# MirceaKitsune/python_raytracer

Measured on AMD Instinct MI355X. Metric: Mrays/s (primary+bounce), higher is better.
Workload: dtype f64; 1 GPU; mods/default 3840x2160 spp8 max_bounces8 (BASELINE config 3/4); width=3840, height=2160, samples=8, primary_rays=62725130, bounce_rays=75192856, partition=(x ^ y) % 1, traversed=True, fast_draws=32, frames_in_flight=1, scene_flow=pre-selected camera chunks (fixture), rng_retraced_rays=0, rng_table=static seeds: draw table + ray table built once before the timed region, reused

## Files before the change

### python_raytracer_amd/_native.py

```python
import ctypes as C
import os
import subprocess

HERE = os.path.dirname(os.path.abspath(__file__))
ROOT = os.path.dirname(HERE)
DIAG = os.environ.get("VRT_DIAG", "0") not in ("", "0")
DIAG_HIST = os.environ.get("VRT_DIAG", "0") == "2"
SO_OVERRIDE = os.environ.get("VRT_SO", "")
SO_PATH = SO_OVERRIDE or os.path.join(HERE, ("_vrt_diaghist.so" if DIAG_HIST else "_vrt_diag.so") if DIAG else "_vrt.so")
UNITS = [os.path.join(HERE, "csrc", f) for f in ("vrt_kernels.hip", "vrt_surface.hip")]
PHYSICS_UNITS = [os.path.join(HERE, "csrc", "vrt_physics.hip")]
PHYSICS_DRAWS_UNITS = [os.path.join(HERE, "csrc", "vrt_physics_draws.hip")]
PHYSICS_RUN_UNITS = [os.path.join(HERE, "csrc", "vrt_physics_run.hip")]
SOURCES = UNITS + PHYSICS_UNITS + PHYSICS_DRAWS_UNITS + PHYSICS_RUN_UNITS + \
    [os.path.join(HERE, "csrc", f) for f in ("vrt_math.h", "vrt_math_consts.h", "vrt_physics_common.h")]
SOURCES.append(os.path.join(ROOT, "include", "vrt.h"))
HIPCC = os.environ.get("HIPCC", "/opt/rocm/bin/hipcc")
HIPCC_FLAGS = ["-O3", "--offload-arch=gfx950", "-ffp-contract=off", "-std=c++17", "-fPIC", "-shared"] + \
    (["-DVRT_DIAG"] if DIAG else []) + (["-DVRT_DIAG_HIST"] if DIAG_HIST else [])

ABI_VERSION = 9
SCENE_TABLE_IS_IDENTITY = 1
SCENE_LAYOUT_DENSE = 2
ERR_WORKSPACE = -3
# ... 291 lines not shown
    L.vrt_diag_launch_census.argtypes = [C.c_int, C.c_char_p, C.c_int, C.POINTER(i64)]
    if L.vrt_abi_version() != ABI_VERSION:
        raise ImportError("python_raytracer_amd/_vrt.so has ABI version %d, expected %d"
                          % (L.vrt_abi_version(), ABI_VERSION))
    _lib = L
    return L


EXPORTS = ["vrt_abi_version", "vrt_status_string", "vrt_last_hip_error", "vrt_device_count", "vrt_release_caches", "vrt_voxel_offset",
           "vrt_max_samples", "vrt_plan_bytes", "vrt_plan_build", "vrt_workspace_bytes", "vrt_render_tile",
           "vrt_views_workspace_bytes", "vrt_render_views",
           "vrt_first_hit", "vrt_first_hit_views_workspace_bytes", "vrt_first_hit_views", "vrt_cast_rays",
           "vrt_shade_workspace_bytes", "vrt_shade_rays", "vrt_path_workspace_bytes", "vrt_path_rays", "vrt_pixel_rays",
           "vrt_draw_table_bytes", "vrt_draw_table_build", "vrt_ray_table_bytes", "vrt_ray_table_build",
           "vrt_pow_memo_create", "vrt_occupancy_build", "vrt_canvas_blit", "vrt_world_tables_bytes", "vrt_world_tables_build",
           "vrt_trace_workspace_bytes", "vrt_trace_rays", "vrt_rng_draws",
           "vrt_synth_volume", "vrt_profile_begin", "vrt_profile_begin_kinds", "vrt_profile_end", "vrt_select_chunks", "vrt_voxelize",
           "vrt_hit_owners", "vrt_hit_surfaces", "vrt_edit_models", "vrt_stamp_model", "vrt_physics_tick",
           "vrt_physics_tick_draws", "vrt_physics_run"]


PLAN_FIELDS = ("launches", "pool", "wt_on", "trav_words", "bm_window", "ct_cells", "n_materials", "dyn_bytes", "static_bytes")
PLAN_PROBE_FIELDS = ("wt_on", "trav_words", "dyn_bytes", "static_bytes", "groups_per_cu")


def last_plan():
    L = lib()
    n = L.vrt_diag_last_plan((C.c_int64 * 1)(), 0)
    if n < 0:
        check(n, "vrt_diag_last_plan")
    buf = (C.c_int64 * n)()
    L.vrt_diag_last_plan(buf, n)
    w = [int(v) for v in buf]
    plan = dict(zip(PLAN_FIELDS, w))
    k = len(PLAN_FIELDS) + 1
    plan["probes"] = [dict(zip(PLAN_PROBE_FIELDS, w[k + 5 * i:k + 5 * i + 5])) for i in range(w[len(PLAN_FIELDS)])]
    return plan


VARIANT_INPUTS = ("record", "list", "list_seed", "pool", "resmode", "deep", "per_pixel", "wt_on", "keys", "trav_words", "bm_window",
                  "big_scene", "tile_heads", "occ", "lookup", "defer_visit")
VARIANT_DEFAULTS = {**dict.fromkeys(VARIANT_INPUTS, 0), "bm_window": -1, "defer_visit": 1}


def march_variant(**inputs):
    unknown = set(inputs) - set(VARIANT_INPUTS)
    if unknown:
        raise TypeError("unknown inputs: %s" % sorted(unknown))
    words = (C.c_int32 * len(VARIANT_INPUTS))(*[int({**VARIANT_DEFAULTS, **inputs}[k]) for k in VARIANT_INPUTS])
    name, effects = C.create_string_buffer(128), (C.c_int32 * 3)()
    status = lib().vrt_diag_march_variant(words, len(VARIANT_INPUTS), name, len(name), effects)
    return (status, name.value.decode(), tuple(effects)) if status == 0 else (status, None, None)


def launch_census():
    L = lib()
    name, count = C.create_string_buffer(128), C.c_int64(0)
    census, row, n = {}, 0, 1
    while row < n:
# ... 16 lines not shown
```

### python_raytracer_amd/csrc/vrt_kernels.hip

```cpp
#include <hip/hip_runtime.h>
#include <stdint.h>
#include <stdio.h>
#include <stdlib.h>
#include <string.h>

#include <atomic>
#include <mutex>
#include <vector>

#include "../../include/vrt.h"
#include "vrt_math.h"

#pragma clang fp contract(off)

#define VRT_WAVE 64
#define VRT_BLOCK 256

static thread_local int g_last_hip_error = 0;
#define HIP_TRY(expr)                                   \
    do {                                                \
        hipError_t e__ = (expr);                        \
        if (e__ != hipSuccess) {                        \
            g_last_hip_error = (int)e__;                \
            return VRT_ERR_HIP;                         \
// ... 832 lines not shown
    double step, life, bounces, energy;
    int nm4x, nm4y, nm4z;
    uint32_t entry;
    uint32_t boff;
    uint32_t color;
    int ndraw, resnaps;
    uint32_t off;
    uint32_t rowi;
    double d0, d1, d2;
    uint32_t view;
};

__device__ __forceinline__ unsigned long long wave_first_u64(unsigned long long v) {
    const unsigned lo = __builtin_amdgcn_readfirstlane((unsigned)v), hi = __builtin_amdgcn_readfirstlane((unsigned)(v >> 32));
    return ((unsigned long long)hi << 32) | lo;
}

enum { LANE_IDLE = 0, LANE_MARCH = 1, LANE_HIT = 2, LANE_ENDED = 3, LANE_ENDED_BROKE = 4, LANE_ENDED_EXHAUSTED = 5 };
__device__ __forceinline__ int opaque_zero() {
    int z = 0;
    asm volatile("" : "+v"(z));
    return z;
}
enum { COLD_POS = 0, COLD_ROT = 3, COLD_DIST_MIN = 7, COLD_POW_Y, COLD_LOD_BOUNCES, COLD_MAX_LIGHT, COLD_MAX_BOUNCES1,
       COLD_SHUTTER, COLD_CS, COLD_INV_CS, COLD_N };
enum { C_LOOKUP = 0, C_NBR, C_CGET, C_HIT, C_ADV, C_NLOCAL };

typedef __attribute__((address_space(3))) uint32_t lds_u32;
typedef __attribute__((address_space(3))) double lds_f64;
typedef __attribute__((address_space(3))) unsigned long long lds_u64;
typedef __attribute__((address_space(3))) char lds_char;

struct MarchCtx {
    const lds_char* tab;
    int tl[3];
    const lds_u32* ct;
    lds_u32* bm;
    const lds_f64* mats;
    const lds_f64* cold;
    lds_u32* tot;
    PowCache pc;
    __amdgpu_buffer_rsrc_t vox;
    unsigned cs4;
    double cs, inv_cs;
    bool kept_cs;
    bool has_bm, tile;

    int td[3];
    int toc[3], oc[3], dm[3];
    const lds_char* wt;
    int wb[3];
    unsigned cs3;
    const lds_char* vw;
};
#define COLD(i) C.cold[(i) + opaque_zero()]
enum { CF_HAS_BM = 1, CF_CT_LDS = 2, CF_CT_IDENTITY = 4, CF_HAS_KEYS = 8, CF_BM_WINDOW = 16 };

#ifdef VRT_DIAG
enum { DG_PASSES = 0, DG_CYC_REFILL, DG_CYC_MARCH, DG_CYC_HIT, DG_CYC_END, DG_ITERS, DG_MARCH_LANES, DG_HIT_EXEC,
       DG_HIT_LANES, DG_END_EXEC, DG_END_LANES, DG_REFILL_EXEC, DG_REFILL_LANES, DG_WAVE_CYCLES, DG_SNAP_ITERS,
       DG_SNAP_LANES, DG_BRICK_VISITS, DG_SWAPS, DG_SWAP_LANES, DG_EVICT_LANES, DG_CYC_SWAP, DG_VOID_LANES,
#ifdef VRT_DIAG_HIST
       DG_NV1, DG_H1 = DG_NV1 + 8, DG_N = DG_H1 + 8
#else
       DG_N
#endif
};
__device__ unsigned long long g_diag[DG_N];
__device__ unsigned long long g_diag_t[5];
#define DG_ADD(idx_, val_)                                                                                      \
    do {                                                                                                        \
        const unsigned long long v_ = (unsigned long long)(val_);   \
        const unsigned long long e_ = __ballot(1);                                                              \
        if ((int)(threadIdx.x & 63) == __ffsll((long long)e_) - 1) dg.acc[idx_] += v_;                           \
    } while (0)
#define DG_TIME() __builtin_amdgcn_s_memtime()
struct DgLane {
    __attribute__((address_space(3))) unsigned long long* acc;
    unsigned brick;
// ... 292 lines not shown
        const RayRecord rec = Q.tab.rec[px];
        ox = rec.ox; oy = rec.oy; oz = rec.oz; ow = rec.ow;
        life = (int)((uint32_t)ray - px * (uint32_t)Q.g.smax) < (int)rec.d0 ? rec.life : -1.0;
        t0 = t1 = t2 = 0.5;
        if (!FH && life >= 0.0) {
            const double* row = Q.draws + rowi * Q.draw_stride + Q.first_draw;
            t0 = row[0];
            t1 = row[1];
            t2 = row[2];
        }
    } else {
        const RayRecord rec = Q.tab.rec[ray];
        life = rec.life; ox = rec.ox; oy = rec.oy; oz = rec.oz; ow = rec.ow;
        t0 = rec.d0; t1 = rec.d1; t2 = rec.d2;
    }
    if (life < 0.0) {
        if (Q.ray_rgba) Q.ray_rgba[ray] = 0;
        if (RECORD && Q.rays) Q.rays[ray].s = -1;
        return false;
    }
    r.off = (uint32_t)off;
    const double cq0 = COLD(COLD_ROT), cq1 = COLD(COLD_ROT + 1), cq2 = COLD(COLD_ROT + 2), cq3 = COLD(COLD_ROT + 3);
    const double dist_min = COLD(COLD_DIST_MIN), cpx = COLD(COLD_POS), cpy = COLD(COLD_POS + 1), cpz = COLD(COLD_POS + 2);
    camera_forward(cq0, cq1, cq2, cq3, ox, oy, oz, ow, r.vx, r.vy, r.vz);
    r.life = life;
    r.px = cpx + r.vx * dist_min;
    r.py = cpy + r.vy * dist_min;
    r.pz = cpz + r.vz * dist_min;
    r.step = 0;
    r.bounces = 0;
    r.energy = 0;
    r.color = 0;
#ifdef VRT_DIAG
    dg.brick = ~0u;
    DG_BRICK();
#endif
    r.nm4x = r.nm4y = r.nm4z = (int)0x80000000u;
    r.entry = 0;
    r.boff = 0;
    r.resnaps = 0;
    r.ndraw = Q.first_draw;
    r.rowi = (uint32_t)rowi;
    r.d0 = t0;
    r.d1 = t1;
    r.d2 = t2;
    if (SNAP) {
        const bool at_origin = r.px == 0.0 && r.py == 0.0 && r.pz == 0.0;
        if (0.0 < life && !at_origin) {
            int fx, fy, fz;
            floor3_i32(r.px, r.py, r.pz, fx, fy, fz);
            resnap_commit<RECORD, true>(Q, C, r, fx, fy, fz, wmin_key, sl, Q.snap_flags);
        }
    }
    return true;
}

template <bool LIST, int SEED, bool FH = false, int PP = 2>
__device__ __forceinline__ bool take_ray_views(const MarchParams& P, const MarchCtx& C, int64_t k, Ray& r) {
    const auto& Q = fresh_args(P);
    const int64_t off = LIST ? (int64_t)Q.list[k] : k;
    const uint32_t bray = (uint32_t)(Q.ray0 + off);
    const uint32_t v = bray / Q.views.view_slots;
    const uint32_t ray = bray - v * Q.views.view_slots;
    const int64_t rowi = LIST ? k : (FH ? 0 : (int64_t)Q.ray_seedidx[ray]);
    if (LIST && SEED != 0) {
        const uint32_t p = ray / (uint32_t)Q.g.smax;
        seed_row<SEED>(Q, Q.g.pixels[2 * (int64_t)p], Q.g.pixels[2 * (int64_t)p + 1], (int)(ray - p * (uint32_t)Q.g.smax), rowi);
    }
    double life, ox, oy, oz, ow, t0, t1, t2;
    if (PP == 1 || (PP == 2 && Q.per_pixel)) {
        const uint32_t px = ray / (uint32_t)Q.g.smax;
        const RayRecord rec = Q.tab.rec[px];
        ox = rec.ox; oy = rec.oy; oz = rec.oz; ow = rec.ow;
        life = (int)(ray - px * (uint32_t)Q.g.smax) < (int)rec.d0 ? rec.life : -1.0;
        t0 = t1 = t2 = 0.5;
        if (!FH && life >= 0.0) {
            const double* row = Q.draws + rowi * Q.draw_stride + Q.first_draw;
// ... 86 lines not shown
#ifdef VRT_DIAG
    if (__ballot(!inside)) { DG_ADD(DG_SNAP_ITERS, 1); DG_ADD(DG_SNAP_LANES, __popcll(__ballot(!inside))); }
#endif
    if (!inside) {
        VRT_MARK("m_resnap");
        const unsigned ux = (unsigned)l4x, uy = (unsigned)l4y, uz = (unsigned)l4z;
        const unsigned umax = ux > uy ? (ux > uz ? ux : uz) : (uy > uz ? uy : uz);
        bool outside = (umax > cs4) | ((ux == cs4) & (r.px != (double)fx)) | ((uy == cs4) & (r.py != (double)fy)) |
                       ((uz == cs4) & (r.pz != (double)fz));
        if (__ballot(l4or == 0x80000000u) != 0ull) {
            if (l4or == 0x80000000u) outside = !(r.px == 0.0 && r.py == 0.0 && r.pz == 0.0);
        }
        if (outside) {
            if constexpr (VIEWS == 3) resnap_cursor(Q, C, r, fx, fy, fz, fl);
            else if constexpr (VIEWS != 0) resnap_commit_views<VIEWS == 1>(Q, C, r, fx, fy, fz, fl);
            else resnap_commit<RECORD, FRESH, DEFER>(Q, C, r, fx, fy, fz, wmin_key, sl, fl, &pend);
            l4x = (int)(((unsigned)fx << 2) + (unsigned)r.nm4x);
            l4y = (int)(((unsigned)fy << 2) + (unsigned)r.nm4y);
            l4z = (int)(((unsigned)fz << 2) + (unsigned)r.nm4z);
            inside = true;
        }
    }
    VRT_MARK("m_entry");
    if (r.entry) {
        VRT_MARK("m_spec");
        const unsigned res = r.entry >> 24;
        const double sd = RESMODE == 0 ? 1.0 : (double)(res ? res : 1u);
        const bool res2 = RESMODE != 0 && res == 2u;
        const unsigned m4 = res2 ? 0x3f8u : 0x3fcu;
        const double magic_r = __hiloint2double(res2 ? 0x43480000 : 0x43380000, 0);
        const unsigned sh_r = res2 ? 3u : 2u;
        const double dvx = RESMODE == 0 ? r.vx : r.vx * sd, dvy = RESMODE == 0 ? r.vy : r.vy * sd,
                     dvz = RESMODE == 0 ? r.vz : r.vz * sd;
        unsigned o[SPEC];
        constexpr bool PIPE = VRT_TAB_PIPELINE && RESMODE != 2;
        uint32_t pt0 = 0, pt1 = 0, pt2 = 0;
        bool pin = inside;
        if (PIPE) {
            const unsigned m0 = RESMODE == 0 ? ~0u : m4;
            pt0 = tab_at(C, 0, (unsigned)l4x & m0);
            pt1 = tab_at(C, 1, (unsigned)l4y & m0);
            pt2 = tab_at(C, 2, (unsigned)l4z & m0);
        } else {
            o[0] = cell_offset<RESMODE>(C, r.entry, r.boff, m4, cs4, r.nm4x, r.nm4y, r.nm4z, l4x, l4y, l4z, inside, true);
        }
        int n_valid = 1;
        constexpr bool CKPT = SPEC == 8 && RESMODE != 2 && LK == 0;
        constexpr int CKPT_AT = 4;
        double cqx = 0, cqy = 0, cqz = 0, cqs = 0;
        {
            double qx = r.px, qy = r.py, qz = r.pz, qs = r.step;
            bool ok = true;
#pragma unroll
            for (int k = 1; k < SPEC; k++) {
                qx += dvx;
                qy += dvy;
                qz += dvz;
                qs += sd;
                int gx, gy, gz, kx, ky, kz;
                if (RESMODE == 0) {
                    floor3_i32(qx, qy, qz, gx, gy, gz);
                    kx = (int)(((unsigned)gx << 2) + (unsigned)r.nm4x);
                    ky = (int)(((unsigned)gy << 2) + (unsigned)r.nm4y);
                    kz = (int)(((unsigned)gz << 2) + (unsigned)r.nm4z);
                } else {
                    floor3_i32_lane(qx, qy, qz, magic_r, gx, gy, gz);
                    kx = (int)(((unsigned)gx << sh_r) + (unsigned)r.nm4x);
                    ky = (int)(((unsigned)gy << sh_r) + (unsigned)r.nm4y);
                    kz = (int)(((unsigned)gz << sh_r) + (unsigned)r.nm4z);
                }
                ok = ok && (qs < r.life) && ((unsigned)(kx | ky | kz) < cs4);
                n_valid += ok ? 1 : 0;
                if (CKPT && k == CKPT_AT) {
                    cqx = qx;
                    cqy = qy;
// ... 83 lines not shown
                            uint64_t* bs = lk.brick_slot;
                            bs[0] = a0.x; bs[1] = a0.y; bs[2] = a1.x; bs[3] = a1.y;
                            bs[4] = a2.x; bs[5] = a2.y; bs[6] = a3.x; bs[7] = a3.y;
                        }
                        const uint64_t cw = lk.brick_slot[widx & 7u];
                        hitmask |= ((unsigned)(cw >> (o[k] & 63u)) & 1u) << k;
                    }
                }
            }
            found = hitmask != 0u;
            if (found) {
                h = __ffs(hitmask) - 1;
                unsigned hoff = o[0];
#pragma unroll
                for (int k = 1; k < SPEC; k++) hoff = (h == k) ? o[k] : hoff;
                r.color |= (unsigned)__builtin_amdgcn_raw_buffer_load_b8(C.vox, hoff, 0, 0) << 24;
            }
        }
        VRT_MARK("m_adv");
        if (DEFER) resnap_finish<DEFER == 2>(Q, C, pend, (unsigned)h, wmin_key);
#ifdef VRT_DIAG_HIST
#pragma unroll
        for (int k = 1; k <= SPEC && k <= 8; k++) {
            DG_ADD(DG_NV1 + k - 1, __popcll(__ballot(n_valid >= k)));
            DG_ADD(DG_H1 + k - 1, __popcll(__ballot(h >= k)));
        }
#endif
        cnt[C_LOOKUP] += h + (found ? 1 : 0);
        cnt[C_ADV] += h;
        int rem = h;
        if (CKPT) {
#ifndef VRT_DIAG
            if (h >= CKPT_AT) {
                r.px = cqx;
                r.py = cqy;
                r.pz = cqz;
                r.step = cqs;
                rem = h - CKPT_AT;
            }
#endif
        }
#pragma unroll
        for (int k = 0; k < SPEC; k++) {
#ifndef VRT_DIAG
            if (CKPT && k >= (CKPT_AT - 1 > SPEC - CKPT_AT ? CKPT_AT - 1 : SPEC - CKPT_AT)) break;
#endif
            if (k < rem) {
                r.step += sd;
                r.px += dvx;
                r.py += dvy;
                r.pz += dvz;
// ... 405 lines not shown
        o.counters[VRT_C_DRAW] = r.ndraw;
        o.counters[VRT_C_ADV] = cnt[C_ADV];
        o.counters[VRT_C_BROKE] = broke;
        o.detail = detail; o.energy = energy; o.step = r.step; o.life = r.life; o.bounces = r.bounces;
        o.pos[0] = r.px; o.pos[1] = r.py; o.pos[2] = r.pz;
        o.vel[0] = r.vx; o.vel[1] = r.vy; o.vel[2] = r.vz;
    }
    lds_u32* col = C.tot + (threadIdx.x & (VRT_TOT_COLS - 1));
#define VRT_TOT_ADD(j, v) __hip_atomic_fetch_add(col + (j) * VRT_TOT_COLS, (uint32_t)(v), __ATOMIC_RELAXED, __HIP_MEMORY_SCOPE_WORKGROUP)
    if (PERRAY) {
        VRT_TOT_ADD(VRT_C_LOOKUP, cnt[C_LOOKUP]);
        VRT_TOT_ADD(VRT_C_NBR, cnt[C_NBR]);
        VRT_TOT_ADD(VRT_C_CHUNK_GET, cnt[C_CGET]);
        VRT_TOT_ADD(VRT_C_HIT, cnt[C_HIT]);
        VRT_TOT_ADD(VRT_C_ADV, cnt[C_ADV]);
    }
    VRT_TOT_ADD(VRT_C_RESNAP, r.resnaps);
    VRT_TOT_ADD(VRT_C_DRAW, r.ndraw);
    VRT_TOT_ADD(VRT_C_BROKE, broke);
    VRT_TOT_ADD(VRT_NCOUNTERS, 1);
#undef VRT_TOT_ADD
}

template <bool W>
struct MarchSharedT {
    unsigned long long stats[VRT_NSTATS];
    unsigned long long pw_keys[VRT_PW_SLOTS];
    unsigned long long pw_vals[VRT_PW_SLOTS];
    uint32_t tab[W ? 4 : 3 * 256];
    uint32_t tot[VRT_NCOUNTERS + 1][VRT_TOT_COLS];
    uint32_t wmin[VRT_BLOCK / VRT_WAVE], wtmp[VRT_BLOCK / VRT_WAVE];
    double cold[COLD_N];
};
typedef MarchSharedT<false> MarchShared;
template <bool W = false, bool TD_ARGS = false>
__device__ __forceinline__ void march_prologue(const MarchParams& P, MarchSharedT<W>& S, unsigned char* s_dyn, MarchCtx& C) {
    double* s_mats = reinterpret_cast<double*>(s_dyn);
    uint32_t* s_ct = reinterpret_cast<uint32_t*>(s_dyn + (size_t)P.n_materials * 64);
    uint32_t* s_trav = s_ct + P.ct_cells;
    for (int i = threadIdx.x; i < P.n_materials * 8; i += VRT_BLOCK) s_mats[i] = P.materials[i];
    for (int i = threadIdx.x; i < P.ct_cells; i += VRT_BLOCK) s_ct[i] = P.chunk_table[i];
    for (int i = threadIdx.x; i < P.trav_words; i += VRT_BLOCK) s_trav[i] = 0u;
    if (threadIdx.x < VRT_BLOCK / VRT_WAVE) S.wmin[threadIdx.x] = 0u;
    for (int i = threadIdx.x; i < VRT_PW_SLOTS; i += VRT_BLOCK) {
        unsigned long long k = 0, v = 0;
        if (P.pow_global) {
            k = __hip_atomic_load(&P.pow_global[i], __ATOMIC_RELAXED, __HIP_MEMORY_SCOPE_AGENT);
            v = __hip_atomic_load(&P.pow_global[VRT_PW_SLOTS + i], __ATOMIC_RELAXED, __HIP_MEMORY_SCOPE_AGENT);
        }
        S.pw_keys[i] = k;
        S.pw_vals[i] = k ? v : 0ull;
    }
    for (int i = threadIdx.x; !W && i < 256; i += VRT_BLOCK) {
        const int c = i < P.cs ? i : 0;
        S.tab[i] = (uint32_t)voxel_offset(P.cs, c, 0, 0);
        S.tab[256 + i] = (uint32_t)voxel_offset(P.cs, 0, c, 0);
        S.tab[512 + i] = (uint32_t)voxel_offset(P.cs, 0, 0, c);
    }
    if (threadIdx.x < VRT_TOT_COLS) {
#pragma unroll
        for (int j = 0; j <= VRT_NCOUNTERS; j++) S.tot[j][threadIdx.x] = 0u;
    }
    if (threadIdx.x < VRT_NSTATS) S.stats[threadIdx.x] = 0;
    if (threadIdx.x == 0) {
        for (int a = 0; a < 3; a++) S.cold[COLD_POS + a] = P.cam.pos[a];
        for (int a = 0; a < 4; a++) S.cold[COLD_ROT + a] = P.cam.rot[a];
        S.cold[COLD_DIST_MIN] = P.st.dist_min;
        S.cold[COLD_POW_Y] = 1 + P.st.falloff;
        S.cold[COLD_LOD_BOUNCES] = P.st.lod_bounces;
        S.cold[COLD_MAX_LIGHT] = P.st.max_light;
        S.cold[COLD_MAX_BOUNCES1] = P.st.max_bounces + 1;
        S.cold[COLD_SHUTTER] = P.st.shutter;
        S.cold[COLD_CS] = (double)P.cs;
        S.cold[COLD_INV_CS] = 1.0 / (double)P.cs;
    }
    C.wt = (const lds_char*)(s_dyn + P.wt_lds_off);
    C.wb[0] = C.wb[1] = C.wb[2] = 0;
    if (W) {
        uint32_t* wt = reinterpret_cast<uint32_t*>(s_dyn + P.wt_lds_off);
        for (int i = threadIdx.x; i < P.wt_words; i += VRT_BLOCK) wt[i] = P.wt_table[i];
        int first = 0;
        for (int a = 0; a < 3; a++) {
            C.wb[a] = 4 * (first + VRT_WT_GUARD - P.wt_min[a]);
            C.tl[a] = 4 * (first + VRT_WT_GUARD);
            first += P.wt_cells[a] + 2 * VRT_WT_GUARD;
        }
        C.tab = C.wt;
    } else {
        C.tab = (const lds_char*)S.tab;
        C.tl[0] = 0;
        C.tl[1] = 1024;
        C.tl[2] = 2048;
    }
    C.cs3 = 1u << (3 * P.cs_shift);
    C.ct = (const lds_u32*)s_ct;
    C.bm = (lds_u32*)s_trav;
    C.mats = (const lds_f64*)s_mats;
// ... 165 lines not shown
    const int64_t count = LIST ? (int64_t)(*P.list_count < P.list_cap ? *P.list_count : P.list_cap) : P.n;
    const int64_t chunk = P.chunk;
    int64_t next = 0, range_end = 0;
    bool more = true;
    if (chunk == 0) {
        const int64_t n_waves = (int64_t)gridDim.x * (VRT_BLOCK / VRT_WAVE);
        const int64_t wave = (int64_t)blockIdx.x * (VRT_BLOCK / VRT_WAVE) + wave_in_block;
        int64_t per = (count + n_waves - 1) / n_waves;
        per = (per + 7) & ~(int64_t)7;
        next = wave * per;
        range_end = next + per < count ? next + per : count;
        more = false;
    }

    Ray r;
    ray_clear(r);
    int state = LANE_IDLE;
    int32_t cnt[C_NLOCAL];
#pragma unroll
    for (int j = 0; j < C_NLOCAL; j++) cnt[j] = 0;
    SeenList<RECORD> sl;
    sl.n = 0;
    uint64_t wmin_key = 0;
    LkState lk = lk_unused();
    if (LK == 2) lk.brick_slot = reinterpret_cast<uint64_t*>(s_dyn + P.brick_lds_off) + 9 * threadIdx.x;
    DG_LANE(dg);
#ifdef VRT_DIAG
    const unsigned long long dg_t_start = __builtin_amdgcn_s_memrealtime();
    unsigned long long dg_t_empty = 0;
    const unsigned long long dg_start = DG_TIME();
#endif

    for (;;) {
#ifdef VRT_DIAG
        DG_ADD(DG_PASSES, 1);
        unsigned long long dg_t0 = DG_TIME();
        {
            const int nidle = __popcll(__ballot(state == LANE_IDLE));
            if (nidle && (next < range_end || more)) { DG_ADD(DG_REFILL_EXEC, 1); DG_ADD(DG_REFILL_LANES, nidle); }
        }
#endif
        if (W && C.has_bm && (!(next < range_end || more) || next < range_end)) {
            if ((threadIdx.x & 63) == 0) S.wtmp[wave_in_block] = (next < range_end || more) ? (uint32_t)(P.ray0 + next) : 0xffffffffu;
            if (state != LANE_IDLE) atomicMin(&S.wtmp[wave_in_block], (uint32_t)(P.ray0 + r.off));
            wmin_key = publish_wave_min(S, wave_in_block, S.wtmp[wave_in_block]);
        }
        unsigned long long idle_mask = __ballot(state == LANE_IDLE);
        while (idle_mask != 0ull && (next < range_end || more)) {
            if (next >= range_end) {
                unsigned long long base = 0;
                if ((threadIdx.x & 63) == 0) base = atomicAdd(P.queue_head, (unsigned long long)chunk);
                base = wave_first_u64(base);
                if ((int64_t)base >= count) {
                    more = false;
#ifdef VRT_DIAG
                    if (!dg_t_empty) dg_t_empty = __builtin_amdgcn_s_memrealtime();
#endif
                    break;
                }
                next = (int64_t)base;
                range_end = next + chunk < count ? next + chunk : count;
            }
            const unsigned rank = __builtin_amdgcn_mbcnt_hi((unsigned)(idle_mask >> 32),
                                                            __builtin_amdgcn_mbcnt_lo((unsigned)idle_mask, 0u));
            const int64_t k = next + rank;
            next += __popcll(idle_mask);
            if (state == LANE_IDLE && k < range_end) {
                sl.n = 0;
                if (take_ray<RECORD, LIST, PERPIX, W, SEED>(P, C, k, r, dg, wmin_key, sl)) {
#pragma unroll
                    for (int j = 0; j < C_NLOCAL; j++) cnt[j] = 0;
                    state = LANE_MARCH;
                }
            }
            idle_mask = __ballot(state == LANE_IDLE);
        }
        if (__ballot(state != LANE_IDLE) == 0ull) break;
        if (!W && C.has_bm) {
            if ((threadIdx.x & 63) == 0) S.wtmp[wave_in_block] = 0xffffffffu;
            if (state != LANE_IDLE) atomicMin(&S.wtmp[wave_in_block], (uint32_t)(P.ray0 + r.off));
            wmin_key = publish_wave_min(S, wave_in_block, S.wtmp[wave_in_block]);
        }
#ifdef VRT_DIAG
        unsigned long long dg_t1 = DG_TIME();
        DG_ADD(DG_CYC_REFILL, dg_t1 - dg_t0);
#endif

        int iters = 0;
        for (;;) {
            const int n_march = (int)__popcll(__ballot(state == LANE_MARCH));
            const int n_hit = (int)__popcll(__ballot(state == LANE_HIT));
            const int n_end = (int)__popcll(__ballot(state >= LANE_ENDED));
            if (n_march == 0 || n_hit >= P.t_hit || n_end >= P.t_end) break;
            if (iters >= P.max_iters && n_hit + n_end > 0) break;
            iters++;
            DG_ADD(DG_ITERS, 1);
            DG_ADD(DG_MARCH_LANES, n_march);
// ... 616 lines not shown
    if (lane < VRT_POOL_SLOTS) pool_state[lane] = (uint32_t)LANE_IDLE;
    __syncthreads();

    const int64_t count = P.n;
    const int64_t chunk = P.chunk > 0 ? P.chunk : VRT_CHUNK;
    const int64_t tail_start = count - (int64_t)gridDim.x * (2 * VRT_BLOCK);
    int64_t next = 0, range_end = 0;
    bool more = true;
    bool tiled = false;
    int ts = 0;
    if constexpr (TILE) {
        tiled = P.tile_heads != nullptr && P.plan_hdr->full_frame != 0;
        unsigned xcc = 0;
        xcc = __builtin_amdgcn_s_getreg((3 << 11) | 20);
        ts = (int)(xcc & 7u);
    }

    Ray r;
    ray_clear(r);
    int state = LANE_IDLE;
    SeenList<false> sl = seen_unused();
    LkState lk = lk_unused();
    uint64_t wmin_key = 0;
    DG_LANE(dg);
#ifdef VRT_DIAG
    const unsigned long long dg_t_start = __builtin_amdgcn_s_memrealtime();
    unsigned long long dg_t_empty = 0;
    const unsigned long long dg_start = DG_TIME();
#endif

    auto refill = [&]() {
        unsigned long long idle_mask = __ballot(state == LANE_IDLE);
#ifdef VRT_DIAG
        DG_ADD(DG_REFILL_EXEC, 1);
        DG_ADD(DG_REFILL_LANES, __popcll(idle_mask));
#endif
        while (idle_mask != 0ull && (next < range_end || more)) {
            if (TILE && next >= range_end && tiled) {
                int64_t first = -1;
                ts = tile_take(P, ts, lane, chunk, first);
                if (first < 0) {
                    more = false;
#ifdef VRT_DIAG
                    if (!dg_t_empty) dg_t_empty = __builtin_amdgcn_s_memrealtime();
#endif
                    break;
                }
                next = first;
                range_end = first + chunk;
            } else if (next >= range_end) {
                unsigned long long base = 0;
                if (lane == 0) base = atomicAdd(P.queue_head, (unsigned long long)chunk);
                base = wave_first_u64(base);
                if ((int64_t)base >= count) {
                    more = false;
#ifdef VRT_DIAG
                    if (!dg_t_empty) dg_t_empty = __builtin_amdgcn_s_memrealtime();
#endif
                    break;
                }
                next = (int64_t)base;
                range_end = next + chunk < count ? next + chunk : count;
            }
            const unsigned rank = __builtin_amdgcn_mbcnt_hi((unsigned)(idle_mask >> 32),
                                                            __builtin_amdgcn_mbcnt_lo((unsigned)idle_mask, 0u));
            const int64_t k = next + rank;
            next += __popcll(idle_mask);
            if (state == LANE_IDLE && k < range_end) {
                SeenList<false> none;
                none.n = 0;
                if (take_ray<false, false, PERPIX, W>(P, C, k, r, dg, W ? wmin_key : 0ull, none)) state = LANE_MARCH;
            }
            idle_mask = __ballot(state == LANE_IDLE);
        }
    };
    constexpr bool PASS_COUNTS = W || VRT_PASS_COUNTS;
    int32_t tot[C_NLOCAL];
#pragma unroll
    for (int j = 0; j < C_NLOCAL; j++) tot[j] = 0;
    constexpr bool FUSE_ENDED = (VRT_POOL_FUSE & 1) != 0, FUSE_HIT = (VRT_POOL_FUSE & 2) != 0;
    unsigned pass = 0;
    int stalled = 0;
    for (;; pass++) {
#ifdef VRT_DIAG
        DG_ADD(DG_PASSES, 1);
#endif
        VRT_MARK("pass");
        if (PASS_COUNTS) {
#pragma unroll
            for (int j = 0; j < C_NLOCAL; j++) tot[j] = 0;
        }
        const int sstate = lane < VRT_POOL_SLOTS ? (int)__hip_atomic_load(pool_state + lane, __ATOMIC_RELAXED, __HIP_MEMORY_SCOPE_WAVEFRONT) : -1;
        const bool lane_i = state == LANE_IDLE;
        const unsigned long long l_m = __ballot(state == LANE_MARCH), l_h = __ballot(state == LANE_HIT),
                                 l_e = __ballot(state >= LANE_ENDED), l_i = __ballot(lane_i);
// ... 1126 lines not shown
    auto pick = [](int env, int dflt, int lo, int hi) { const int v = env >= 0 ? env : dflt; return v < lo ? lo : (v > hi ? hi : v); };
    P.t_hit = pick(h, big_scene ? 48 : 40, 1, cap);
    P.t_end = pick(e, big_scene ? 32 : 60, 1, cap);
    P.pool_swap_min = pick(sw, big_scene ? 4 : 8, 1, 64);
    P.pool_refill_min = pick(rf, 8, 1, 64);
    P.pool_keep = pick(kp, 40, 1, 64);
    P.max_iters = pick(it, big_scene ? 5 : 3, 1, 64);
}
static inline size_t march_lds(MarchParams& P, bool bricks, bool pool) {
    P.snap_flags = (P.trav_words != 0 ? CF_HAS_BM | (P.bm_window >= 0 ? CF_BM_WINDOW : 0) : 0) | (P.ct_cells != 0 ? CF_CT_LDS : 0) | (P.ct_identity != 0 ? CF_CT_IDENTITY : 0) |
                   (P.t_keys != nullptr ? CF_HAS_KEYS : 0);
    size_t n = (size_t)P.n_materials * 64 + (size_t)P.ct_cells * 4 + (size_t)P.trav_words * 4;
    n = (n + 15) & ~(size_t)15;
    P.wt_lds_off = (int32_t)n;
    if (P.wt_on)
        for (int a = 0; a < 3; a++) n += ((size_t)P.wt_cells[a] + 2 * VRT_WT_GUARD) * 4;
    P.brick_lds_off = (int32_t)n;
    if (bricks) n += (size_t)VRT_BLOCK * 9 * 8;
    P.pool_lds_off = (int32_t)n;
    if (pool) n += (size_t)(VRT_BLOCK / VRT_WAVE) * VRT_POOL_WAVE_BYTES;
    return n + 16;
}
#define VRT_PLAN_PROBES 4
#define VRT_PLAN_WORDS (10 + 5 * VRT_PLAN_PROBES)
struct PlanRecord {
    int64_t w[VRT_PLAN_WORDS];
    bool probes_fresh;
};
static thread_local PlanRecord g_plan = {{0}, false};
static inline int64_t plan_static_bytes(bool w) {
    return (int64_t)(((w ? sizeof(MarchSharedT<true>) : sizeof(MarchShared)) + 15) & ~(size_t)15);
}
static void plan_probe(const MarchParams& P, size_t dyn, bool w, int nb) {
    if (!g_plan.probes_fresh) {
        g_plan.probes_fresh = true;
        g_plan.w[9] = 0;
    }
    if (g_plan.w[9] >= VRT_PLAN_PROBES) return;
    int64_t* q = g_plan.w + 10 + 5 * g_plan.w[9]++;
    q[0] = P.wt_on;
    q[1] = P.trav_words;
    q[2] = (int64_t)dyn;
    q[3] = plan_static_bytes(w);
    q[4] = nb;
}
static void plan_record(const MarchParams& P, size_t dyn, bool pool) {
    if (!g_plan.probes_fresh) g_plan.w[9] = 0;
    g_plan.probes_fresh = false;
    g_plan.w[0]++;
    g_plan.w[1] = pool ? 1 : 0;
    g_plan.w[2] = P.wt_on;
    g_plan.w[3] = P.trav_words;
    g_plan.w[4] = P.bm_window;
    g_plan.w[5] = P.ct_cells;
    g_plan.w[6] = P.n_materials;
    g_plan.w[7] = (int64_t)dyn;
    g_plan.w[8] = plan_static_bytes(P.wt_on != 0);
}
static int pool_blocks_per_cu(size_t dyn, bool w) {
    static std::mutex mu;
    static size_t seen_dyn[16];
    static int seen_n[16], n_seen = 0;
    const size_t key = dyn * 2 + (w ? 1 : 0);
    std::lock_guard<std::mutex> lock(mu);
    for (int i = 0; i < n_seen; i++)
        if (seen_dyn[i] == key) return seen_n[i];
    int nb = 0;
    hipError_t e = w ? hipOccupancyMaxActiveBlocksPerMultiprocessor(&nb, march_pool_kernel<8, 1, 0, true>, VRT_BLOCK, dyn)
                     : hipOccupancyMaxActiveBlocksPerMultiprocessor(&nb, march_pool_kernel<VRT_SPEC_DEEP, 1>, VRT_BLOCK, dyn);
    if (e != hipSuccess) nb = 0;
    if (env_int("VRT_POOL_VERBOSE", 0))
        fprintf(stderr, "vrt: march_pool_kernel%s: %zu + %zu bytes of LDS per workgroup -> %d workgroups per CU\n", w ? " (look-ahead)" : "",
                w ? sizeof(MarchSharedT<true>) : sizeof(MarchShared), dyn, nb);
    if (n_seen < 16) {
        seen_dyn[n_seen] = key;
        seen_n[n_seen++] = nb;
    }
    return nb;
}
static bool pool_fits(MarchParams& P, bool w) {
// ... 145 lines not shown
#define VRT_BY_RES(resmode, K) ((resmode) == 0 ? (MarchFn)K(VRT_SPEC_DEEP, 0) : (resmode) == 1 ? (MarchFn)K(VRT_SPEC_DEEP, 1) : (MarchFn)K(VRT_SPEC, 2))
struct ByResInstance { MarchFn fn; const char* name; };
#define VRT_CENSUS_ROW(...) {(MarchFn)&__VA_ARGS__, VRT_STR(__VA_ARGS__)},
#define VRT_CENSUS_BY_RES(K, ...) VRT_CENSUS_ROW(K<VRT_SPEC_DEEP,0,__VA_ARGS__>) VRT_CENSUS_ROW(K<VRT_SPEC_DEEP,1,__VA_ARGS__>) VRT_CENSUS_ROW(K<VRT_SPEC,2,__VA_ARGS__>)
#define VRT_CENSUS_FIRST_HIT(S, R, V) VRT_CENSUS_ROW(first_hit_kernel<S,R,1,V>) VRT_CENSUS_ROW(first_hit_kernel<S,R,0,V>)
#define VRT_CENSUS_FIRST_HITS(V) VRT_CENSUS_FIRST_HIT(VRT_SPEC_DEEP, 0, V) VRT_CENSUS_FIRST_HIT(VRT_SPEC_DEEP, 1, V) VRT_CENSUS_FIRST_HIT(VRT_SPEC, 2, V)
static const ByResInstance g_by_res_instances[] = {
    VRT_CENSUS_BY_RES(march_views_kernel, false,0)
    VRT_CENSUS_ROW(march_views_kernel<VRT_SPEC,2,true,1>) VRT_CENSUS_ROW(march_views_kernel<VRT_SPEC,2,true,2>)
    VRT_CENSUS_FIRST_HITS(false) VRT_CENSUS_FIRST_HITS(true)
    VRT_CENSUS_ROW(cast_kernel<VRT_SPEC_DEEP,0>) VRT_CENSUS_ROW(cast_kernel<VRT_SPEC_DEEP,1>) VRT_CENSUS_ROW(cast_kernel<VRT_SPEC,2>)
    VRT_CENSUS_BY_RES(shade_kernel, true) VRT_CENSUS_BY_RES(shade_kernel, false)};
#undef VRT_CENSUS_FIRST_HITS
#undef VRT_CENSUS_FIRST_HIT
#undef VRT_CENSUS_BY_RES
#undef VRT_CENSUS_ROW
#define VRT_N_BY_RES_INSTANCES ((int)(sizeof g_by_res_instances / sizeof g_by_res_instances[0]))
static std::atomic<int64_t> g_by_res_launches[VRT_N_BY_RES_INSTANCES];
static inline void launch_by_res(MarchFn fn, int grid, size_t lds, hipStream_t stream, const MarchParams& P) {
    for (int i = 0; i < VRT_N_BY_RES_INSTANCES; i++)
        if (g_by_res_instances[i].fn == fn) g_by_res_launches[i].fetch_add(1, std::memory_order_relaxed);
    launch_fn(fn, grid, lds, stream, P);
}
static int launch_march(MarchParams P, int grid, int resmode, bool deep, bool pool, bool record, bool list, hipStream_t stream) {
    const bool big_scene = big_voxels(P.vox_bytes);
    const MarchChoiceIn in = {record, list, P.list_seed, pool, resmode, deep, P.per_pixel, P.wt_on, P.t_keys != nullptr, P.trav_words, P.bm_window,
                              big_scene, P.tile_heads != nullptr, P.occ != nullptr, lookup_mode(), env_int("VRT_DEFER_VISIT", 1)};
    MarchChoice c;
    if (march_choose(in, c) != VRT_OK) return VRT_ERR_ARG;
    P.wt_on = c.wt_on;
    P.trav_words = c.trav_words;
    if (!c.keep_tile_heads) P.tile_heads = nullptr;
    if (pool) pool_policy(P, big_scene);
    const size_t lds = march_lds(P, c.k->v.lk == 2, pool);
    if (!list) plan_record(P, lds, pool);
    g_march_launches[c.k - g_march_instances].fetch_add(1, std::memory_order_relaxed);
    launch_fn(c.k->fn, grid, lds, stream, P);
    return VRT_OK;
}
static inline bool march_wt_ok(const MarchParams& P, int resmode, bool deep) { return P.wt_on && march_eight(resmode, deep, lookup_mode()); }
static inline int res_mode(const vrt_scene* sc) {
    static int force = -2;
    if (force == -2) force = env_int("VRT_RESMODE", -1);
    if (force >= 0 && force <= 2) return force == 2 ? 2 : (sc->max_resolution >= 1 && sc->max_resolution <= force + 1 ? force : 2);
    return sc->max_resolution == 1 ? 0 : (sc->max_resolution == 2 ? 1 : 2);
}

struct ViewOrigins { int32_t o[64][4]; };
__global__ void __launch_bounds__(64) views_setup_kernel(const vrt_camera* cams, ViewOrigins org, int v0, int n, double* view_tab) {
    const int t = threadIdx.x;
    if (t >= n) return;
    const double* c = reinterpret_cast<const double*>(cams + v0 + t);
    double* out = view_tab + (int64_t)(v0 + t) * VRT_VIEW_WORDS;
    for (int i = 0; i < 8; i++) out[i] = c[i];
    *reinterpret_cast<int4*>(out + 8) = make_int4(org.o[t][0], org.o[t][1], org.o[t][2], 0);
}
static void setup_views(const vrt_camera* d_cams, const vrt_traversed* traversed, int n_views, int chunk_size, double* view_tab,
// ... 1212 lines not shown
```

Measured before the change: 29590 Mrays/s.

## Pre-snap camera chunk entry per block and merge void-chunk skips into spec loop

Each workgroup now computes the camera's starting chunk entry, offsets and traversal cell once in the prologue and stores them in LDS. Fresh primary rays copy this state instead of doing their own initial snap, and a wave-level atomicMin records the first visiting ray for traversal keys. Separately, empty-chunk lanes now take a void step through the same speculative march block as occupied lanes rather than a separate path, which is meant to cut divergence. This adds per-block prologue work, more LDS, and a ballot per refill, and it relies on host checks (dist_min == 0, camera inside the traversal grid) to stay correct.

Result: no change. 29840 Mrays/s (median of 6 runs) (+0.9%).

```diff
diff --git a/python_raytracer_amd/_native.py b/python_raytracer_amd/_native.py
--- a/python_raytracer_amd/_native.py
+++ b/python_raytracer_amd/_native.py
@@ -337,6 +337,7 @@
 
 PLAN_FIELDS = ("launches", "pool", "wt_on", "trav_words", "bm_window", "ct_cells", "n_materials", "dyn_bytes", "static_bytes")
 PLAN_PROBE_FIELDS = ("wt_on", "trav_words", "dyn_bytes", "static_bytes", "groups_per_cu")
+PLAN_PROBES = 4
 
 
 def last_plan():
@@ -350,6 +351,7 @@
     plan = dict(zip(PLAN_FIELDS, w))
     k = len(PLAN_FIELDS) + 1
     plan["probes"] = [dict(zip(PLAN_PROBE_FIELDS, w[k + 5 * i:k + 5 * i + 5])) for i in range(w[len(PLAN_FIELDS)])]
+    plan["presnap"] = w[k + 5 * PLAN_PROBES] if n > k + 5 * PLAN_PROBES else 0
     return plan
 
 
diff --git a/python_raytracer_amd/csrc/vrt_kernels.hip b/python_raytracer_amd/csrc/vrt_kernels.hip
--- a/python_raytracer_amd/csrc/vrt_kernels.hip
+++ b/python_raytracer_amd/csrc/vrt_kernels.hip
@@ -878,8 +878,15 @@
     asm volatile("" : "+v"(z));
     return z;
 }
+#ifndef VRT_VOID_MERGE
+#define VRT_VOID_MERGE 1
+#endif
+#ifndef VRT_PRESNAP
+#define VRT_PRESNAP 1
+#endif
 enum { COLD_POS = 0, COLD_ROT = 3, COLD_DIST_MIN = 7, COLD_POW_Y, COLD_LOD_BOUNCES, COLD_MAX_LIGHT, COLD_MAX_BOUNCES1,
        COLD_SHUTTER, COLD_CS, COLD_INV_CS, COLD_N };
+enum { COLD_SNAP = COLD_CS, SNAP_NM4 = 0, SNAP_ENTRY = 3, SNAP_RESNAPS, SNAP_TCI, SNAP_N };
 enum { C_LOOKUP = 0, C_NBR, C_CGET, C_HIT, C_ADV, C_NLOCAL };
 
 typedef __attribute__((address_space(3))) uint32_t lds_u32;
@@ -910,7 +917,7 @@
     const lds_char* vw;
 };
 #define COLD(i) C.cold[(i) + opaque_zero()]
-enum { CF_HAS_BM = 1, CF_CT_LDS = 2, CF_CT_IDENTITY = 4, CF_HAS_KEYS = 8, CF_BM_WINDOW = 16 };
+enum { CF_HAS_BM = 1, CF_CT_LDS = 2, CF_CT_IDENTITY = 4, CF_HAS_KEYS = 8, CF_BM_WINDOW = 16, CF_PRESNAP = 32 };
 
 #ifdef VRT_DIAG
 enum { DG_PASSES = 0, DG_CYC_REFILL, DG_CYC_MARCH, DG_CYC_HIT, DG_CYC_END, DG_ITERS, DG_MARCH_LANES, DG_HIT_EXEC,
@@ -1249,6 +1256,7 @@
     r.off = (uint32_t)off;
     const double cq0 = COLD(COLD_ROT), cq1 = COLD(COLD_ROT + 1), cq2 = COLD(COLD_ROT + 2), cq3 = COLD(COLD_ROT + 3);
     const double dist_min = COLD(COLD_DIST_MIN), cpx = COLD(COLD_POS), cpy = COLD(COLD_POS + 1), cpz = COLD(COLD_POS + 2);
+    constexpr bool PRE = VRT_PRESNAP && !RECORD && !LIST && !SNAP && SEED == 0 && !FH;
     camera_forward(cq0, cq1, cq2, cq3, ox, oy, oz, ow, r.vx, r.vy, r.vz);
     r.life = life;
     r.px = cpx + r.vx * dist_min;
@@ -1266,6 +1274,15 @@
     r.entry = 0;
     r.boff = 0;
     r.resnaps = 0;
+    if (PRE) {
+        const lds_u32* sw = (const lds_u32*)(C.cold + (COLD_SNAP + opaque_zero()));
+        r.nm4x = (int)sw[SNAP_NM4];
+        r.nm4y = (int)sw[SNAP_NM4 + 1];
+        r.nm4z = (int)sw[SNAP_NM4 + 2];
+        r.entry = sw[SNAP_ENTRY];
+        r.boff = ((r.entry & 0xffffffu) - 1u) << (3 * Q.cs_shift);
+        r.resnaps = 0.0 < life ? (int)sw[SNAP_RESNAPS] : 0;
+    }
     r.ndraw = Q.first_draw;
     r.rowi = (uint32_t)rowi;
     r.d0 = t0;
@@ -1280,6 +1297,18 @@
         }
     }
     return true;
+}
+
+template <class PT>
+__device__ __forceinline__ void presnap_visit(const PT& Q, const MarchCtx& C, bool fresh_live, uint32_t off, uint32_t& wrec) {
+    const unsigned long long lm = __ballot(fresh_live);
+    if (lm == 0ull) return;
+    const uint32_t first = (uint32_t)__builtin_amdgcn_readlane((int)off, __ffsll((long long)lm) - 1);
+    if (fresh_live && off == first && first < wrec) {
+        const int tci = (int)((const lds_u32*)(C.cold + (COLD_SNAP + opaque_zero())))[SNAP_TCI];
+        if (tci >= 0) atomicMin((unsigned long long*)&Q.t_keys[tci], (unsigned long long)(Q.ray0 + first) << 12);
+    }
+    wrec = first < wrec ? first : wrec;
 }
 
 template <bool LIST, int SEED, bool FH = false, int PP = 2>
@@ -1412,27 +1441,47 @@
         }
     }
     VRT_MARK("m_entry");
-    if (r.entry) {
+    constexpr bool MERGE = VRT_VOID_MERGE && LK == 0;
+    const bool present = r.entry != 0u;
+    double vstep = 1.0;
+    if (MERGE && !present) {
+        VRT_MARK("m_void");
+#ifdef VRT_DIAG
+        DG_ADD(DG_VOID_LANES, __popcll(__ballot(1)));
+#endif
+        const double mn = min3_f64(r.px, r.py, r.pz);
+        const double t = mn + (double)st.chunk_radius;
+        const double inv_cs = C.kept_cs ? C.inv_cs : COLD(COLD_INV_CS), csd = C.kept_cs ? C.cs : COLD(COLD_CS);
+        const double md = t - __builtin_floor(t * inv_cs) * csd;
+        vstep = 1 + __builtin_fabs((double)st.chunk_radius - md);
+    }
+    if (MERGE || present) {
         VRT_MARK("m_spec");
         const unsigned res = r.entry >> 24;
-        const double sd = RESMODE == 0 ? 1.0 : (double)(res ? res : 1u);
+        const bool skip = MERGE && !present;
+        const double sd = skip ? vstep : (RESMODE == 0 ? 1.0 : (double)(res ? res : 1u));
         const bool res2 = RESMODE != 0 && res == 2u;
         const unsigned m4 = res2 ? 0x3f8u : 0x3fcu;
         const double magic_r = __hiloint2double(res2 ? 0x43480000 : 0x43380000, 0);
         const unsigned sh_r = res2 ? 3u : 2u;
-        const double dvx = RESMODE == 0 ? r.vx : r.vx * sd, dvy = RESMODE == 0 ? r.vy : r.vy * sd,
-                     dvz = RESMODE == 0 ? r.vz : r.vz * sd;
+        double dvx = RESMODE == 0 ? r.vx : r.vx * sd, dvy = RESMODE == 0 ? r.vy : r.vy * sd,
+               dvz = RESMODE == 0 ? r.vz : r.vz * sd;
+        if (RESMODE == 0 && skip) {
+            dvx = r.vx * sd;
+            dvy = r.vy * sd;
+            dvz = r.vz * sd;
+        }
         unsigned o[SPEC];
         constexpr bool PIPE = VRT_TAB_PIPELINE && RESMODE != 2;
         uint32_t pt0 = 0, pt1 = 0, pt2 = 0;
-        bool pin = inside;
+        bool pin = inside && !skip;
         if (PIPE) {
             const unsigned m0 = RESMODE == 0 ? ~0u : m4;
             pt0 = tab_at(C, 0, (unsigned)l4x & m0);
             pt1 = tab_at(C, 1, (unsigned)l4y & m0);
             pt2 = tab_at(C, 2, (unsigned)l4z & m0);
         } else {
-            o[0] = cell_offset<RESMODE>(C, r.entry, r.boff, m4, cs4, r.nm4x, r.nm4y, r.nm4z, l4x, l4y, l4z, inside, true);
+            o[0] = cell_offset<RESMODE>(C, r.entry, r.boff, m4, cs4, r.nm4x, r.nm4y, r.nm4z, l4x, l4y, l4z, inside && !skip, !skip);
         }
         int n_valid = 1;
         constexpr bool CKPT = SPEC == 8 && RESMODE != 2 && LK == 0;
@@ -1440,7 +1489,7 @@
         double cqx = 0, cqy = 0, cqz = 0, cqs = 0;
         {
             double qx = r.px, qy = r.py, qz = r.pz, qs = r.step;
-            bool ok = true;
+            bool ok = !skip;
 #pragma unroll
             for (int k = 1; k < SPEC; k++) {
                 qx += dvx;
@@ -1570,11 +1619,11 @@
 #ifdef VRT_DIAG_HIST
 #pragma unroll
         for (int k = 1; k <= SPEC && k <= 8; k++) {
-            DG_ADD(DG_NV1 + k - 1, __popcll(__ballot(n_valid >= k)));
-            DG_ADD(DG_H1 + k - 1, __popcll(__ballot(h >= k)));
-        }
-#endif
-        cnt[C_LOOKUP] += h + (found ? 1 : 0);
+            DG_ADD(DG_NV1 + k - 1, __popcll(__ballot(!skip && n_valid >= k)));
+            DG_ADD(DG_H1 + k - 1, __popcll(__ballot(!skip && h >= k)));
+        }
+#endif
+        cnt[C_LOOKUP] += skip ? 0 : h + (found ? 1 : 0);
         cnt[C_ADV] += h;
         int rem = h;
         if (CKPT) {
@@ -2026,6 +2075,29 @@
 #undef VRT_TOT_ADD
 }
 
+__device__ __noinline__ void presnap_words(kernarg_ptr p, lds_u32* out) {
+    const auto& Q = *p;
+    int nm4[3] = {(int)0x80000000u, (int)0x80000000u, (int)0x80000000u}, tci = -1;
+    uint32_t entry = 0u, resnaps = 0u;
+    const int fl = Q.snap_flags;
+    if (VRT_PRESNAP && (fl & CF_PRESNAP) != 0) {
+        int cc[3];
+        for (int a = 0; a < 3; a++) {
+            cc[a] = (int)__builtin_floor(Q.cam.pos[a]) >> Q.cs_shift;
+            nm4[a] = -(cc[a] << (Q.cs_shift + 2));
+        }
+        entry = chunk_entry_i(Q, (const lds_u32*)nullptr, cc[0] - Q.origin_c[0], cc[1] - Q.origin_c[1], cc[2] - Q.origin_c[2],
+                              Q.dims[0], Q.dims[1], Q.dims[2], false, (fl & (CF_CT_LDS | CF_CT_IDENTITY)) == CF_CT_IDENTITY);
+        tci = trav_cell((fl & CF_HAS_KEYS) != 0, cc[0], cc[1], cc[2], Q.t_origin_c[0], Q.t_origin_c[1], Q.t_origin_c[2],
+                        Q.t_dims[0], Q.t_dims[1], Q.t_dims[2]);
+        resnaps = 1u;
+    }
+    for (int a = 0; a < 3; a++) out[SNAP_NM4 + a] = (uint32_t)nm4[a];
+    out[SNAP_ENTRY] = entry;
+    out[SNAP_RESNAPS] = resnaps;
+    out[SNAP_TCI] = (uint32_t)tci;
+}
+
 template <bool W>
 struct MarchSharedT {
     unsigned long long stats[VRT_NSTATS];
@@ -2034,9 +2106,11 @@
     uint32_t tab[W ? 4 : 3 * 256];
     uint32_t tot[VRT_NCOUNTERS + 1][VRT_TOT_COLS];
     uint32_t wmin[VRT_BLOCK / VRT_WAVE], wtmp[VRT_BLOCK / VRT_WAVE];
-    double cold[COLD_N];
+    double cold[W ? COLD_N : COLD_SNAP];
+    uint32_t snap[W ? 2 : SNAP_N];
 };
 typedef MarchSharedT<false> MarchShared;
+static_assert(offsetof(MarchShared, snap) == offsetof(MarchShared, cold) + 8 * COLD_SNAP, "take_ray finds the snap words behind the cold scalars");
 template <bool W = false, bool TD_ARGS = false>
 __device__ __forceinline__ void march_prologue(const MarchParams& P, MarchSharedT<W>& S, unsigned char* s_dyn, MarchCtx& C) {
     double* s_mats = reinterpret_cast<double*>(s_dyn);
@@ -2075,8 +2149,12 @@
         S.cold[COLD_MAX_LIGHT] = P.st.max_light;
         S.cold[COLD_MAX_BOUNCES1] = P.st.max_bounces + 1;
         S.cold[COLD_SHUTTER] = P.st.shutter;
-        S.cold[COLD_CS] = (double)P.cs;
-        S.cold[COLD_INV_CS] = 1.0 / (double)P.cs;
+        if constexpr (W) {
+            S.cold[COLD_CS] = (double)P.cs;
+            S.cold[COLD_INV_CS] = 1.0 / (double)P.cs;
+        } else {
+            presnap_words(&fresh_args(P), (lds_u32*)S.snap);
+        }
     }
     C.wt = (const lds_char*)(s_dyn + P.wt_lds_off);
     C.wb[0] = C.wb[1] = C.wb[2] = 0;
@@ -2288,6 +2366,9 @@
     SeenList<RECORD> sl;
     sl.n = 0;
     uint64_t wmin_key = 0;
+    constexpr bool PRE = VRT_PRESNAP && !RECORD && !LIST && !W;
+    uint32_t wrec = 0xffffffffu;
+    asm volatile("" : "+v"(wrec));
     LkState lk = lk_unused();
     if (LK == 2) lk.brick_slot = reinterpret_cast<uint64_t*>(s_dyn + P.brick_lds_off) + 9 * threadIdx.x;
     DG_LANE(dg);
@@ -2331,14 +2412,17 @@
                                                             __builtin_amdgcn_mbcnt_lo((unsigned)idle_mask, 0u));
             const int64_t k = next + rank;
             next += __popcll(idle_mask);
+            bool got = false;
             if (state == LANE_IDLE && k < range_end) {
                 sl.n = 0;
                 if (take_ray<RECORD, LIST, PERPIX, W, SEED>(P, C, k, r, dg, wmin_key, sl)) {
 #pragma unroll
                     for (int j = 0; j < C_NLOCAL; j++) cnt[j] = 0;
                     state = LANE_MARCH;
+                    got = true;
                 }
             }
+            if (PRE) presnap_visit(fresh_args(P), C, got && 0.0 < r.life, r.off, wrec);
             idle_mask = __ballot(state == LANE_IDLE);
         }
         if (__ballot(state != LANE_IDLE) == 0ull) break;
@@ -3001,6 +3085,9 @@
     SeenList<false> sl = seen_unused();
     LkState lk = lk_unused();
     uint64_t wmin_key = 0;
+    constexpr bool PRE = VRT_PRESNAP && !W;
+    uint32_t wrec = 0xffffffffu;
+    asm volatile("" : "+v"(wrec));
     DG_LANE(dg);
 #ifdef VRT_DIAG
     const unsigned long long dg_t_start = __builtin_amdgcn_s_memrealtime();
@@ -3045,11 +3132,16 @@
                                                             __builtin_amdgcn_mbcnt_lo((unsigned)idle_mask, 0u));
             const int64_t k = next + rank;
             next += __popcll(idle_mask);
+            bool got = false;
             if (state == LANE_IDLE && k < range_end) {
                 SeenList<false> none;
                 none.n = 0;
-                if (take_ray<false, false, PERPIX, W>(P, C, k, r, dg, W ? wmin_key : 0ull, none)) state = LANE_MARCH;
+                if (take_ray<false, false, PERPIX, W>(P, C, k, r, dg, W ? wmin_key : 0ull, none)) {
+                    state = LANE_MARCH;
+                    got = true;
+                }
             }
+            if (PRE) presnap_visit(fresh_args(P), C, got && 0.0 < r.life, r.off, wrec);
             idle_mask = __ballot(state == LANE_IDLE);
         }
     };
@@ -4222,7 +4314,7 @@
     return n + 16;
 }
 #define VRT_PLAN_PROBES 4
-#define VRT_PLAN_WORDS (10 + 5 * VRT_PLAN_PROBES)
+#define VRT_PLAN_WORDS (10 + 5 * VRT_PLAN_PROBES + 5)
 struct PlanRecord {
     int64_t w[VRT_PLAN_WORDS];
     bool probes_fresh;
@@ -4256,6 +4348,7 @@
     g_plan.w[6] = P.n_materials;
     g_plan.w[7] = (int64_t)dyn;
     g_plan.w[8] = plan_static_bytes(P.wt_on != 0);
+    g_plan.w[10 + 5 * VRT_PLAN_PROBES] = (P.snap_flags & CF_PRESNAP) != 0 ? 1 : 0;
 }
 static int pool_blocks_per_cu(size_t dyn, bool w) {
     static std::mutex mu;
@@ -4447,6 +4540,17 @@
         if (g_by_res_instances[i].fn == fn) g_by_res_launches[i].fetch_add(1, std::memory_order_relaxed);
     launch_fn(fn, grid, lds, stream, P);
 }
+static bool march_presnap(const MarchParams& P, const MarchVariant& v) {
+    if (!VRT_PRESNAP || v.record || v.list || v.w || P.g.pixels == nullptr) return false;
+    if (!(P.st.dist_min == 0.0)) return false;
+    if (P.cam.pos[0] == 0.0 && P.cam.pos[1] == 0.0 && P.cam.pos[2] == 0.0) return false;
+    if (P.t_keys == nullptr) return true;
+    for (int a = 0; a < 3; a++) {
+        const int c = ((int)floor(P.cam.pos[a]) >> P.cs_shift) - P.t_origin_c[a];
+        if ((unsigned)c >= (unsigned)P.t_dims[a]) return false;
+    }
+    return true;
+}
 static int launch_march(MarchParams P, int grid, int resmode, bool deep, bool pool, bool record, bool list, hipStream_t stream) {
     const bool big_scene = big_voxels(P.vox_bytes);
     const MarchChoiceIn in = {record, list, P.list_seed, pool, resmode, deep, P.per_pixel, P.wt_on, P.t_keys != nullptr, P.trav_words, P.bm_window,
@@ -4458,6 +4562,7 @@
     if (!c.keep_tile_heads) P.tile_heads = nullptr;
     if (pool) pool_policy(P, big_scene);
     const size_t lds = march_lds(P, c.k->v.lk == 2, pool);
+    if (march_presnap(P, c.k->v)) P.snap_flags |= CF_PRESNAP;
     if (!list) plan_record(P, lds, pool);
     g_march_launches[c.k - g_march_instances].fetch_add(1, std::memory_order_relaxed);
     launch_fn(c.k->fn, grid, lds, stream, P);
```
